# Cappucciyes/ViT-With-OpenCL

Hardware: AMD Instinct MI355X
Metric: images/sec ViT-B/16 224x224 bs512 (higher is better)
Workload: dtype f32

## Files before the change

vit-with-opencl_amd/csrc/ViT_hip.c:

```c
#include "ViT_opencl.h"
#include "vit_ingest.h"
#include "vit_plan.h"

#include <math.h>
#include <pthread.h>
#include <stddef.h>
#include <stdint.h>
#include <stdio.h>
#include <stdlib.h>
#include <string.h>
#include <time.h>

#define TRY(expr)                 \
    do {                          \
        int try_rc_ = (expr);     \
        if (try_rc_ != 0) {       \
            rc = try_rc_;         \
            goto fail;            \
        }                         \
    } while (0)

enum { DESC_RING = 8 };

enum { FEAT_NONE, FEAT_DEVICE, FEAT_HOST };

struct staged
{
    void *dev, *pinned[2];
    char *host;
    size_t per_image;
};

struct vit_hip_ctx
{
    vit_config cfg;
    int device;
    int max_batch;
    int n_tensors;
    vh_stream_t stream;

    struct vit_plan plan;

    void *slab[N_SLABS];
    float **w;
    struct operand *op;

    float *x;
    float *y;
    float *attn;
    float *qkv;
    float *hid;
    float *stats;
    float *cls;
    float *d_logits;
    float *d_probs;
    float *d_images[2];
    float *h_images[2];
    float *h_logits[2];
    float *h_probs[2];
    vh_stream_t copy_stream;
    vh_event_t up_done[2], comp_done[2], out_done[2];

    vh_resize_desc *h_desc[DESC_RING];
    vh_resize_desc *d_desc[DESC_RING];
    vh_event_t desc_done[DESC_RING];
    int desc_live[DESC_RING];
    int desc_next;

    struct feature_req
    {
        int form;
        vit_feature_spec spec;
        int layer[4];
        vit_feature_buffers out;
        struct staged st[2];
    } feat;

    struct topk_req
    {
        int form;
        vit_topk_spec spec;
        vit_topk_buffers out;
        struct staged st[2];
    } topk;

    struct attn_req
    {
        int form;
        vit_attn_spec spec;
        int layer[4];
        vit_attn_buffers out;
        struct staged st[2];
    } amap;
    const struct attn_req *attn_serving;

    vh_event_t *prof_ev;
    int *prof_class;
    int prof_cap;
    int prof_used;
    unsigned prof_mask;
};

static int prof_begin(vit_hip_ctx *ctx, vh_stream_t s, int op_class)
{
    if (!ctx->prof_ev || ctx->prof_used >= ctx->prof_cap)
        return -1;
    if (ctx->prof_mask && !(ctx->prof_mask & (1u << op_class)))
        return -1;
    const int slot = ctx->prof_used++;
    ctx->prof_class[slot] = op_class;
    vh_event_record(ctx->prof_ev[2 * slot], s);
    return slot;
}

// ... 34 lines not shown
const vit_config *vit_hip_config(const vit_hip_ctx *ctx) { return &ctx->cfg; }
int vit_hip_device(const vit_hip_ctx *ctx) { return ctx->device; }
float *vit_hip_logits_buffer(vit_hip_ctx *ctx) { return ctx->d_logits; }
vh_stream_t vit_hip_stream(const vit_hip_ctx *ctx) { return ctx->stream; }
int vit_hip_max_batch(const vit_hip_ctx *ctx) { return ctx->max_batch; }
const float *vit_hip_weight(const vit_hip_ctx *ctx, int idx)
{
    return (idx >= 0 && idx < ctx->n_tensors) ? ctx->w[idx] : NULL;
}

static int staged_alloc(const vit_hip_ctx *ctx, struct staged *st)
{
    const size_t bytes = (size_t)ctx->max_batch * st->per_image;
    int rc = vh_malloc(&st->dev, bytes);
    for (int slot = 0; slot < 2 && rc == 0; ++slot)
        rc = vh_host_alloc(&st->pinned[slot], bytes);
    return rc;
}

static void staged_release(struct staged *st)
{
    if (st->dev) vh_free(st->dev);
    st->dev = NULL;
    for (int slot = 0; slot < 2; ++slot) {
        if (st->pinned[slot]) vh_host_free(st->pinned[slot]);
        st->pinned[slot] = NULL;
    }
}

static int staged_d2h(const vit_hip_ctx *ctx, const struct staged *st, int slot, int m)
{
    return vh_d2h(st->pinned[slot], st->dev, (size_t)m * st->per_image, ctx->stream);
}

static void staged_scatter(const struct staged *st, int slot, int first, int m)
{
    memcpy(st->host + (size_t)first * st->per_image, st->pinned[slot], (size_t)m * st->per_image);
}

static void request_release(struct staged st[2])
{
    staged_release(&st[0]);
    staged_release(&st[1]);
}

void vit_hip_destroy(vit_hip_ctx *ctx)
{
    if (!ctx)
        return;
    if (ctx->stream) {
        vh_set_device(ctx->device);
        vh_stream_sync(ctx->stream);
    }
    prof_release(ctx);
    request_release(ctx->feat.st);
    request_release(ctx->topk.st);
    request_release(ctx->amap.st);
    for (int i = 0; i < N_SLABS; ++i)
        if (ctx->slab[i])
            vh_free(ctx->slab[i]);
    float *dev[] = {ctx->x, ctx->y, ctx->attn, ctx->qkv, ctx->hid, ctx->stats,
                    ctx->cls, ctx->d_logits, ctx->d_probs, ctx->d_images[0], ctx->d_images[1]};
    for (size_t i = 0; i < sizeof(dev) / sizeof(dev[0]); ++i)
        if (dev[i])
            vh_free(dev[i]);
    float *host[] = {ctx->h_images[0], ctx->h_images[1], ctx->h_logits[0], ctx->h_logits[1],
                     ctx->h_probs[0], ctx->h_probs[1]};
    for (size_t i = 0; i < sizeof(host) / sizeof(host[0]); ++i)
        if (host[i])
            vh_host_free(host[i]);
    for (int i = 0; i < DESC_RING; ++i) {
        if (ctx->d_desc[i]) vh_free(ctx->d_desc[i]);
        if (ctx->h_desc[i]) vh_host_free(ctx->h_desc[i]);
        if (ctx->desc_done[i]) vh_event_destroy(ctx->desc_done[i]);
    }
    for (int i = 0; i < 2; ++i) {
        if (ctx->up_done[i]) vh_event_destroy(ctx->up_done[i]);
        if (ctx->comp_done[i]) vh_event_destroy(ctx->comp_done[i]);
        if (ctx->out_done[i]) vh_event_destroy(ctx->out_done[i]);
    }
    if (ctx->copy_stream)
        vh_stream_destroy(ctx->copy_stream);
    if (ctx->stream)
        vh_stream_destroy(ctx->stream);
    free(ctx->w);
    free(ctx->op);
    free(ctx);
}

static float **layer_tensors(const vit_hip_ctx *ctx, int l) { return ctx->w + 4 + 12 * l; }

static int alloc_weights(vit_hip_ctx *ctx)
{
    int rc = 0;
    for (int i = 0; i < N_SLABS; ++i)
        if (ctx->plan.slab_bytes[i])
            TRY(vh_malloc(&ctx->slab[i], ctx->plan.slab_bytes[i]));
    plan_layout(&ctx->plan, &ctx->cfg, ctx->slab, ctx->w, ctx->op, NULL);
    return 0;
fail:
    return rc;
}

static int fill_weights(vit_hip_ctx *ctx, const Network *networks)
{
    int rc = 0;
// ... 1049 lines not shown
        return 1;
    TRY(vh_set_device(ctx->device));
    TRY(vh_stream_sync(ctx->stream));
    prof_release(ctx);
    if (max_forwards <= 0)
        return 0;
    const int per_forward = 1 + 7 * ctx->cfg.depth + 3 + 4 + 1 + 4;
    ctx->prof_cap = per_forward * max_forwards;
    ctx->prof_ev = (vh_event_t *)calloc((size_t)2 * ctx->prof_cap, sizeof(vh_event_t));
    ctx->prof_class = (int *)calloc((size_t)ctx->prof_cap, sizeof(int));
    if (!ctx->prof_ev || !ctx->prof_class) {
        prof_release(ctx);
        return 4;
    }
    for (int i = 0; i < 2 * ctx->prof_cap; ++i)
        TRY(vh_event_create(&ctx->prof_ev[i]));
    return 0;
fail:
    prof_release(ctx);
    return rc;
}

int vit_hip_profile_select(vit_hip_ctx *ctx, unsigned op_mask)
{
    if (!ctx)
        return 1;
    ctx->prof_mask = op_mask;
    return 0;
}

int vit_hip_profile_read(vit_hip_ctx *ctx, double ms_sum[VIT_OP_COUNT], long launches[VIT_OP_COUNT])
{
    int rc = 0;
    if (!ctx || !ms_sum || !launches)
        return 1;
    TRY(vh_set_device(ctx->device));
    for (int k = 0; k < VIT_OP_COUNT; ++k) {
        ms_sum[k] = 0.0;
        launches[k] = 0;
    }
    for (int i = 0; i < ctx->prof_used; ++i) {
        float ms = 0.0f;
        TRY(vh_event_sync(ctx->prof_ev[2 * i + 1]));
        TRY(vh_event_elapsed_ms(&ms, ctx->prof_ev[2 * i], ctx->prof_ev[2 * i + 1]));
        ms_sum[ctx->prof_class[i]] += ms;
        launches[ctx->prof_class[i]] += 1;
    }
    ctx->prof_used = 0;
    return 0;
fail:
    return rc;
}

static void scatter_outputs(vit_hip_ctx *ctx, int slot, int first, int m, const struct staged *const *arrays, int n_arrays, float **probs)
{
    const size_t NC = (size_t)ctx->cfg.num_classes;
    for (int a = 0; a < n_arrays; ++a)
        staged_scatter(arrays[a], slot, first, m);
    if (probs)
        for (int i = 0; i < m; ++i)
            memcpy(probs[first + i], ctx->h_probs[slot] + (size_t)i * NC, NC * sizeof(float));
}

struct gather_job
{
    char *dst;
    const struct ingest_src *src;
    const struct ingest_plan *plan;
    int first, count;
    int base;
    size_t per_image;
};

static void *gather_worker(void *arg)
{
    const struct gather_job *j = (const struct gather_job *)arg;
    for (int i = j->first; i < j->first + j->count; ++i) {
        if (j->plan) {
            ingest_pack(j->dst, j->plan, j->src, i);
            continue;
        }
        const void *from = j->src->kind == INGEST_F32 ? (const void *)j->src->host_f32[j->base + i].data
                                                      : (const void *)(j->src->u8 + (size_t)(j->base + i) * j->per_image);
        memcpy(j->dst + (size_t)i * j->per_image, from, j->per_image);
    }
    return NULL;
}

static void gather_images(void *dst, const struct ingest_src *src, const struct ingest_plan *plan, int base, int m, size_t per_image)
{
    enum { MAX_THREADS = 8 };
    int nt = m / 16;
    if (nt > MAX_THREADS)
        nt = MAX_THREADS;
    struct gather_job jobs[MAX_THREADS];
    pthread_t tid[MAX_THREADS];
    int started = 0;
    if (nt < 2) {
        struct gather_job all = {.dst = (char *)dst, .src = src, .plan = plan, .first = 0, .count = m, .base = base, .per_image = per_image};
        gather_worker(&all);
        return;
    }
    const int per = (m + nt - 1) / nt;
    for (int t = 0; t < nt; ++t) {
        const int first = t * per, count = first >= m ? 0 : (m - first < per ? m - first : per);
        jobs[t] = (struct gather_job){.dst = (char *)dst, .src = src, .plan = plan, .first = first, .count = count, .base = base, .per_image = per_image};
        if (count == 0)
            break;
        if (t == nt - 1 || pthread_create(&tid[started], NULL, gather_worker, &jobs[t]) != 0)
            gather_worker(&jobs[t]);
        else
            ++started;
    }
    for (int t = 0; t < started; ++t)
        pthread_join(tid[t], NULL);
}

static int forward_pipelined(vit_hip_ctx *ctx, const struct ingest_src *src, struct ingest_plan *plan, int n, float *logits, float **probs,
                             int form)
{
    int rc = 0;
    const struct feature_req *fr;
    const struct topk_req *tk;
    const struct attn_req *ar;
    if (armed_requests(ctx, "forward", form, &fr, &tk, &ar))
        return 1;
    TRY(vh_set_device(ctx->device));
    const vit_config *c = &ctx->cfg;
    const size_t bytes = (size_t)c->in_chans * c->img_size * c->img_size * (src->kind == INGEST_F32 ? sizeof(float) : 1);
    const size_t NC = (size_t)c->num_classes;
    const struct staged logits_st = {ctx->d_logits, {ctx->h_logits[0], ctx->h_logits[1]}, (char *)logits, NC * sizeof(float)};
    const struct staged *arrays[7];
    int n_arrays = 0;
    if (logits)
        arrays[n_arrays++] = &logits_st;
    for (int a = 0; a < 6; ++a) {
        const struct staged *st = a < 2 ? (fr ? &fr->st[a] : NULL) : a < 4 ? (tk ? &tk->st[a - 2] : NULL) : (ar ? &ar->st[a - 4] : NULL);
        if (st && st->dev)
            arrays[n_arrays++] = st;
    }

    int prev_first = 0, prev_m = 0, k = 0;
    for (int first = 0, m = 0; first < n; first += m, ++k) {
        const int s = k & 1;
        struct ingest_src dev = *src;
        dev.on_device = 1;
        m = (n - first < ctx->max_batch) ? n - first : ctx->max_batch;
        size_t up = (size_t)m * bytes;
        int jobs = m;
        switch (src->kind) {
        case INGEST_F32:
            dev.host_f32 = NULL;
            dev.f32 = ctx->d_images[s];
            break;
        case INGEST_U8:
            dev.u8 = (const unsigned char *)ctx->d_images[s];
            break;
        default:
            m = ingest_plan_chunk(plan, src, first, n, (const unsigned char *)ctx->d_images[s]);
            up = plan->bytes;
            jobs = plan->n_src;
            dev.items = plan->items;
        }
        if (m <= 0) {
            rc = vh_set_error(1, "forward: an image does not fit a staging slot");
            goto fail;
        }
        gather_images(ctx->h_images[s], src, plan, first, jobs, bytes);
        if (k >= 2)
            TRY(vh_stream_wait_event(ctx->copy_stream, ctx->comp_done[s]));
        TRY(vh_h2d(ctx->d_images[s], ctx->h_images[s], up, ctx->copy_stream));
        TRY(vh_event_record(ctx->up_done[s], ctx->copy_stream));

        TRY(vh_stream_wait_event(ctx->stream, ctx->up_done[s]));
        TRY(forward_device(ctx, &dev, m, ctx->d_logits, probs ? ctx->d_probs : NULL, ctx->stream, fr, tk, ar));
        TRY(vh_event_record(ctx->comp_done[s], ctx->stream));
        int a = 0;
        if (logits)
            TRY(staged_d2h(ctx, arrays[a++], s, m));
        if (probs)
            TRY(vh_d2h(ctx->h_probs[s], ctx->d_probs, (size_t)m * NC * sizeof(float), ctx->stream));
        for (; a < n_arrays; ++a)
            TRY(staged_d2h(ctx, arrays[a], s, m));
        TRY(vh_event_record(ctx->out_done[s], ctx->stream));

        if (k >= 1) {
            TRY(vh_event_sync(ctx->out_done[s ^ 1]));
            scatter_outputs(ctx, s ^ 1, prev_first, prev_m, arrays, n_arrays, probs);
        }
        prev_first = first;
        prev_m = m;
    }
    TRY(vh_event_sync(ctx->out_done[(k - 1) & 1]));
    scatter_outputs(ctx, (k - 1) & 1, prev_first, prev_m, arrays, n_arrays, probs);
    return 0;
fail:
    vh_stream_sync(ctx->copy_stream);
    vh_stream_sync(ctx->stream);
    return rc;
}

static int forward_host_images(vit_hip_ctx *ctx, const ImageData *images, int n, float *logits, float **probs, int form)
{
    if (!ctx || !images || n <= 0)
        return 1;
    const vit_config *c = &ctx->cfg;
    for (int i = 0; i < n; ++i)
        if (!images[i].data || images[i].c != c->in_chans || images[i].h != c->img_size ||
            images[i].w != c->img_size)
            return 5;
    const struct ingest_src src = {.kind = INGEST_F32, .host_f32 = images};
    return forward_pipelined(ctx, &src, NULL, n, logits, probs, form);
}

int vit_hip_forward(vit_hip_ctx *ctx, const ImageData *images, int n, float *logits, float **probs)
{
    return forward_host_images(ctx, images, n, logits, probs, FEAT_HOST);
}

static int forward_host_u8(vit_hip_ctx *ctx, const char *who, const struct ingest_src *src, int n, float *logits, float **probs)
{
    if (source_check(who, ctx, src, n))
        return 1;
    struct ingest_plan *plan = NULL;
    if (src->kind != INGEST_U8) {
        const struct ingest_model model = model_of(ctx);
        if (!(plan = ingest_plan_new(&model, src->kind)))
            return ingest_refuse(who, "out of host memory");
    }
    const int rc = forward_pipelined(ctx, src, plan, n, logits, probs, FEAT_HOST);
    ingest_plan_free(plan);
    return rc;
}

int vit_hip_forward_u8(vit_hip_ctx *ctx, const unsigned char *images, int n, int layout,
                       const vit_pixel_norm *norm, float *logits, float **probs)
{
    const struct ingest_src src = {.kind = INGEST_U8, .u8 = images, .layout = layout, .norm = norm};
    return forward_host_u8(ctx, "vit_hip_forward_u8", &src, n, logits, probs);
}

int vit_hip_forward_u8_resized(vit_hip_ctx *ctx, const vit_image_u8 *images, int n, int layout, const vit_resize_crop *rc,
                               const vit_pixel_norm *norm, float *logits, float **probs)
{
    const struct ingest_src src = {.kind = INGEST_U8_RESIZED, .images = images, .rc = rc, .layout = layout, .norm = norm};
    return forward_host_u8(ctx, "vit_hip_forward_u8_resized", &src, n, logits, probs);
}
// ... 287 lines not shown
```

vit-with-opencl_amd/csrc/vit_plan.c:

```c
#include "vit_plan.h"
#include "vit_ingest.h"

#include <stdio.h>
#include <stdlib.h>
#include <string.h>

void plan_env_parse(struct plan_env *env, const char *const v[PLAN_ENV_COUNT])
{
    const char *const p = v[PLAN_ENV_PRECISION], *const fold = v[PLAN_ENV_LN_FOLD], *const attn = v[PLAN_ENV_ATTN];
    env->precision = (p && p[0] == 'b') ? VIT_PRECISION_BF16_GEMM
                   : (p && strncmp(p, "fp16x2", 6) == 0) ? VIT_PRECISION_F32_FP16X2
                   : (p && strncmp(p, "fp8", 3) == 0) ? VIT_PRECISION_FP8_GEMM : VIT_PRECISION_F32;
    env->p3_off = v[PLAN_ENV_P3] && v[PLAN_ENV_P3][0] == '0';
    env->fp32_native = v[PLAN_ENV_GEMM_FP32] && v[PLAN_ENV_GEMM_FP32][0] == 'n';
    env->ln_fold = (fold && fold[0] == '0') ? 0 : (fold && fold[0] == '1') ? 1 : -1;
    env->last_layer_cls = v[PLAN_ENV_LAST_LAYER] && strcmp(v[PLAN_ENV_LAST_LAYER], "cls") == 0;
    env->attn_long = attn && strcmp(attn, "long") == 0;
    env->attn_tiled = attn && attn[0] == 't';
}

void plan_env_read(struct plan_env *env)
{
    const char *const values[PLAN_ENV_COUNT] = {getenv("VIT_HIP_PRECISION"), getenv("VIT_HIP_P3"), getenv("VIT_HIP_GEMM_FP32"),
                                                getenv("VIT_HIP_LN_FOLD"), getenv("VIT_HIP_LAST_LAYER"), getenv("VIT_HIP_ATTN")};
    plan_env_parse(env, values);
}

static size_t max_of(size_t a, size_t b) { return a > b ? a : b; }

size_t plan_cls_only_scratch(const vit_config *cfg, int n, size_t off[3])
{
    const size_t rows = (size_t)n, E = (size_t)cfg->embed_dim, F = (size_t)cfg->mlp_hidden;
    size_t o[3];
    o[0] = align_up(rows * E * 4, 256);
    o[1] = o[0] + align_up(rows * E * 6, 256);
    o[2] = o[1] + align_up(rows * E * 6, 256);
    if (off)
        memcpy(off, o, sizeof o);
    return o[2] + rows * F * 6;
}

static void *place(void *slab, size_t *off, size_t bytes)
{
    void *p = slab ? (char *)slab + *off : NULL;
    *off += align_up(bytes, 256);
    return p;
}

void plan_layout(const struct vit_plan *plan, const vit_config *cfg, void *const slabs[N_SLABS], float **w, struct operand *op,
                 size_t bytes[N_SLABS])
{
    void *const none[N_SLABS] = {NULL};
    void *const *slab = slabs ? slabs : none;
    struct operand unplaced_op;
    size_t off[N_SLABS] = {0};
    for (int i = 0; i < vit_config_num_tensors(cfg); ++i) {
        float *p = (float *)place(slab[SLAB_F32], &off[SLAB_F32], vit_config_tensor_size(cfg, i) * sizeof(float));
        if (slabs)
            w[i] = p;
    }
    for (int m = 0; m < 4 * cfg->depth; ++m) {
        struct operand *o = slabs ? &op[m] : &unplaced_op;
        const size_t cnt = vit_config_tensor_size(cfg, plan_operand_tensor(m));
        o->w = place(slab[SLAB_OPERAND], &off[SLAB_OPERAND], cnt * (size_t)plan->operand_bytes);
        if (plan->operand_scales)
            o->scales = place(slab[SLAB_OPERAND], &off[SLAB_OPERAND], cnt / 32);
        if (plan->ln_fold && m % 2 == 0) {
            const size_t nb = vit_config_tensor_size(cfg, plan_operand_tensor(m) + 1) * sizeof(float);
            o->colsum = (float *)place(slab[SLAB_FOLD], &off[SLAB_FOLD], nb);
            o->bias_folded = (float *)place(slab[SLAB_FOLD], &off[SLAB_FOLD], nb);
        }
    }
    place(slab[SLAB_CONV], &off[SLAB_CONV],
          (size_t)vh_patch_planes_k(cfg->in_chans, cfg->patch_size) * (size_t)cfg->embed_dim * 2 * (size_t)plan->conv_parts);
    if (bytes)
        memcpy(bytes, off, sizeof(off));
}

static void plan_arena(struct vit_plan *plan, const vit_config *cfg, int max_batch)
{
    const size_t E = (size_t)cfg->embed_dim, F = (size_t)cfg->mlp_hidden, act = (size_t)plan->act_bytes, n = (size_t)max_batch;
    const size_t rows = n * (size_t)plan->tokens, grid = (size_t)(cfg->img_size / cfg->patch_size);
    const size_t img = (size_t)cfg->in_chans * cfg->img_size * cfg->img_size;
    const int fp8 = plan->precision == VIT_PRECISION_FP8_GEMM, resizes = cfg->in_chans <= 4;
    const int planes_path = plan->use_p3 || plan->precision == VIT_PRECISION_BF16_GEMM || fp8;
    size_t b;

    plan->x_bytes = rows * E * sizeof(float);

    b = rows * E * act;
    if (fp8) {
        plan->e_scales_off = align_up(rows * E, 256);
// ... 108 lines not shown
```

vit-with-opencl_amd/csrc/vit_plan.h:

```cpp
#ifndef VIT_PLAN_H
#define VIT_PLAN_H

#include "ViT_opencl.h"

#include <stddef.h>

struct operand
{
    void *w;
    void *scales;
    float pair_scale;
    float *colsum, *bias_folded;
};

enum { SLAB_F32, SLAB_OPERAND, SLAB_CONV, SLAB_FOLD, N_SLABS };

enum { ATTN_STREAMING, ATTN_HD64, ATTN_HD80, ATTN_LONG };

enum { STREAMING_MAX_TOKENS = 512 };

enum { MAX_DEPTH = 256, MAX_TENSORS = 4 + 12 * MAX_DEPTH + 4 };

static inline int plan_operand_tensor(int m)
{
    static const int big[4] = {2, 4, 8, 10};
    return 4 + 12 * (m / 4) + big[m % 4];
}

struct plan_env
{
    int precision;
    int p3_off;
    int fp32_native;
    int ln_fold;
    int last_layer_cls;
    int attn_long;
    int attn_tiled;
};
enum { PLAN_ENV_PRECISION, PLAN_ENV_P3, PLAN_ENV_GEMM_FP32, PLAN_ENV_LN_FOLD, PLAN_ENV_LAST_LAYER, PLAN_ENV_ATTN, PLAN_ENV_COUNT };
void plan_env_parse(struct plan_env *env, const char *const values[PLAN_ENV_COUNT]);
void plan_env_read(struct plan_env *env);

struct vit_plan
{
    int precision;
    int ln_fold;
    int use_p3;
    int cls_only_last;
    int attn_form;
    int fp32_native;
    int attn_rows_streaming;
    int tokens;
    int qkv_form;
    int weight_planes;
    int operand_bytes;
    int operand_scales;
    int conv_parts;
    int planes_patch_embed;
    int act_bytes;
    int cls_only_ok;
    size_t slab_bytes[N_SLABS];
    size_t x_bytes, y_bytes, attn_bytes, qkv_bytes, ws_bytes, stats_bytes;
    size_t crop_off;
    size_t e_scales_off, hid_scales_off;
};

int plan_make(struct vit_plan *plan, const vit_config *cfg, int n_tensors, int max_batch, int precision, int ln_fold,
              const struct plan_env *env);

void plan_layout(const struct vit_plan *plan, const vit_config *cfg, void *const slabs[N_SLABS], float **w, struct operand *op,
                 size_t bytes[N_SLABS]);

size_t plan_cls_only_scratch(const vit_config *cfg, int n, size_t off[3]);

#endif
```

vit-with-opencl_amd/csrc/attention_p3.hip:

```cpp
#include "kernelHandler.h"
#include "vit_kernels.h"
#include "fp32_split.h"
#include "gemm_common.h"

namespace {

constexpr int HD = 64;
constexpr int MAX_LDS = 160 * 1024;
constexpr int MAX_ROWS = 208;

typedef const __attribute__((address_space(1))) void *gptr_t;
typedef __attribute__((address_space(3))) void *lptr_t;
typedef short s16x4 __attribute__((ext_vector_type(4)));

template <int NKT, int NPL, int OUTK>
__global__ __launch_bounds__(64 * NKT) void attention_p3_kernel(const char *__restrict__ qkv3, char *__restrict__ out3,
                                                               unsigned char *__restrict__ out_scales,
                                                               int T, int E, int H, int n_items, int RB)
{
    static_assert((NPL == 3 && OUTK == 3) || (NPL == 1 && (OUTK == 4 || OUTK == 0 || OUTK == 8)), "parts / output kind");
    typedef typename PartT<NPL>::type part_t;
    constexpr int NT = NPL == 3 ? 6 : 1;
    extern __shared__ __attribute__((aligned(16))) char smem[];
    const int slot = 2 * NPL * RB * 64;
    char *Kb = smem, *Vb = smem + slot;

    const int tid = threadIdx.x, lane = tid & 63;
    const int wave = __builtin_amdgcn_readfirstlane(tid >> 6);
    const int lr = lane & 31, lh = lane >> 5;
    const int E32 = E >> 5, rb16 = RB >> 4, pieces = 2 * NPL * rb16;
    const size_t prow = (size_t)(n_items / H) * T;

    auto dma = [&](int item, int which , char *dst) {
        const int b = item / H, h = item - b * H;
        const int ks0 = which * E32 + 2 * h;
        for (int p = wave; p < pieces; p += NKT) {
            const int gp = p / rb16, rb = p - gp * rb16;
            const int r = 16 * rb + (lane >> 2);
            int c = lane & 3;
            if (which == 1)
                c ^= swz64(lane >> 4);
            const char *src = qkv3 + ((size_t)(ks0 * NPL + gp) * prow + (size_t)b * T + min(r, T - 1)) * 64 + 16 * c;
            __builtin_amdgcn_global_load_lds((gptr_t)src, (lptr_t)(dst + p * 1024), 16, 0, 0);
        }
    };

    const int q = wave * 32 + lr;
    part_t qp[HD / 16][NPL];
    auto load_q = [&](int item) {
        const int b = item / H, h = item - b * H;
        const size_t row = (size_t)b * T + min(q, T - 1);
#pragma unroll
        for (int g = 0; g < HD / 16; ++g)
#pragma unroll
            for (int pl = 0; pl < NPL; ++pl)
                qp[g][pl] = __builtin_bit_cast(part_t, *reinterpret_cast<const f32x4 *>(
                                qkv3 + ((size_t)((2 * h + (g >> 1)) * NPL + pl) * prow + row) * 64 + 16 * (2 * (g & 1) + lh)));
    };

    int kofs[2], kofs_last[2];
    {
        const int rl = min(32 * (NKT - 1) + lr, RB - 1);
#pragma unroll
        for (int gl = 0; gl < 2; ++gl) {
            kofs[gl] = lr * 64 + 16 * ((2 * gl + lh) ^ swz64(lr >> 2));
            kofs_last[gl] = rl * 64 + 16 * ((2 * gl + lh) ^ swz64(rl >> 2));
        }
    }
    const int vofs = (4 * lh + ((lane & 15) >> 2)) * 64 + ((lane & 16) + 4 * (lane & 3)) * 2;

    int item = blockIdx.x;
    if (item >= n_items)
        return;
    load_q(item);
    dma(item, 1, Kb);
    __syncthreads();

    for (; item < n_items; item += gridDim.x) {
        const int b = item / H, h = item - b * H;
        const int next = item + gridDim.x;
        dma(item, 2, Vb);

        f32x16 s[NKT];
        part_t kp[3][NPL];
        auto read_k = [&](part_t (&k3)[NPL], int f) {
            const int j = f / (HD / 16), g = f % (HD / 16);
#pragma unroll
            for (int o = 0; o < NPL; ++o) {
                const int pl = (NPL - o) % NPL;
                const char *base = Kb + ((g >> 1) * NPL + pl) * RB * 64;
                k3[pl] = __builtin_bit_cast(part_t, (j < NKT - 1)
                    ? *reinterpret_cast<const f32x4 *>(base + kofs[g & 1] + j * 32 * 64)
                    : *reinterpret_cast<const f32x4 *>(base + kofs_last[g & 1]));
            }
        };
        read_k(kp[0], 0);
        if (NKT * (HD / 16) > 1)
            read_k(kp[1], 1);
#pragma unroll
        for (int f = 0; f < NKT * (HD / 16); ++f) {
            const int j = f / (HD / 16), g = f % (HD / 16);
            if (g == 0) {
#pragma unroll
                for (int r = 0; r < 16; ++r)
                    s[j][r] = 0.0f;
            }
            if (f + 2 < NKT * (HD / 16))
                read_k(kp[(f + 2) % 3], f + 2);
#pragma unroll
            for (int t = 0; t < NT; ++t)
                s[j] = mfma_part(kp[f % 3][term_w<NPL>(t)], qp[g][term_a<NPL>(t)], s[j]);
            if (NPL == 3) {
#pragma unroll
                for (int r = 0; r < 3; ++r) {
                    __builtin_amdgcn_sched_group_barrier(0x100, 1, 0);
                    __builtin_amdgcn_sched_group_barrier(0x008, 2, 0);
                }
                __builtin_amdgcn_sched_barrier(0);
            }
        }

        __syncthreads();
        if (next < n_items) {
            dma(next, 1, Kb);
            load_q(next);
        }

#pragma unroll
        for (int r = 0; r < 16; ++r) {
            const int key = 32 * (NKT - 1) + (r & 3) + 8 * (r >> 2) + 4 * lh;
            s[NKT - 1][r] = key < T ? s[NKT - 1][r] : -INFINITY;
        }
        float mx = -INFINITY;
#pragma unroll
        for (int j = 0; j < NKT; ++j)
#pragma unroll
            for (int r = 0; r < 16; ++r)
                mx = fmaxf(mx, s[j][r]);
        mx = fmaxf(mx, __shfl_xor(mx, 32));
        const float c1 = 1.44269504088896340736f / sqrtf((float)HD);
        const float c2 = -mx * c1;
        float sum = 0.0f;
#pragma unroll
        for (int j = 0; j < NKT; ++j)
#pragma unroll
            for (int r = 0; r < 16; ++r) {
                const float e = __builtin_amdgcn_exp2f(__builtin_fmaf(s[j][r], c1, c2));
                s[j][r] = e;
                sum += e;
            }
        sum += __shfl_xor(sum, 32);
        const float inv_sum = 1.0f / sum;
#pragma unroll
        for (int j = 0; j < NKT; ++j)
#pragma unroll
            for (int r = 0; r < 16; ++r)
                s[j][r] = s[j][r] * inv_sum;

        f32x16 o[2];
#pragma unroll
        for (int r = 0; r < 16; ++r) {
            o[0][r] = 0.0f;
            o[1][r] = 0.0f;
        }
        part_t vq[2][NPL], pp[NPL];
        auto read_v = [&](part_t (&v3)[NPL], int f) {
            const int j = f >> 2, t = (f >> 1) & 1, dt = f & 1;
            const int r0 = (j == NKT - 1) ? min(32 * j + 16 * t, RB - 16) : 32 * j + 16 * t;
#pragma unroll
            for (int o3 = 0; o3 < NPL; ++o3) {
                const int pl = (NPL - o3) % NPL;
                const char *vp = Vb + (dt * NPL + pl) * RB * 64 + r0 * 64 + vofs;
                const s16x4 lo = __builtin_amdgcn_ds_read_tr16_b64_v4i16((__attribute__((address_space(3))) s16x4 *)(vp));
                const s16x4 hi = __builtin_amdgcn_ds_read_tr16_b64_v4i16((__attribute__((address_space(3))) s16x4 *)(vp + 8 * 64));
                typedef short s16x8 __attribute__((ext_vector_type(8)));
                v3[pl] = __builtin_bit_cast(part_t, s16x8{lo[0], lo[1], lo[2], lo[3], hi[0], hi[1], hi[2], hi[3]});
            }
        };
        read_v(vq[0], 0);
#pragma unroll
        for (int f = 0; f < 4 * NKT; ++f) {
            const int j = f >> 2, t = (f >> 1) & 1, dt = f & 1;
            if (f + 1 < 4 * NKT)
                read_v(vq[(f + 1) & 1], f + 1);
            if (dt == 0)
                split_parts(f32x4{s[j][8 * t], s[j][8 * t + 1], s[j][8 * t + 2], s[j][8 * t + 3]},
                            f32x4{s[j][8 * t + 4], s[j][8 * t + 5], s[j][8 * t + 6], s[j][8 * t + 7]}, pp);
            if (!(j == NKT - 1 && 32 * j + 16 * t >= T)) {
#pragma unroll
                for (int tt = 0; tt < NT; ++tt)
                    o[dt] = mfma_part(vq[f & 1][term_w<NPL>(tt)], pp[term_a<NPL>(tt)], o[dt]);
            }
        }

        if (q < T) {
            typedef unsigned u32x2 __attribute__((ext_vector_type(2)));
            typedef unsigned u32x4 __attribute__((ext_vector_type(4)));
            constexpr int OPL = OUTK == 3 ? 3 : 1;
#pragma unroll
            for (int dt = 0; dt < 2; ++dt) {
                if (OUTK == 0) {
                    float *row = reinterpret_cast<float *>(out3) + ((size_t)b * T + q) * E + h * HD + 32 * dt + 4 * lh;
#pragma unroll
                    for (int g = 0; g < 4; ++g)
                        *reinterpret_cast<f32x4 *>(row + 8 * g) = f32x4{o[dt][4 * g], o[dt][4 * g + 1], o[dt][4 * g + 2], o[dt][4 * g + 3]};
                    continue;
                }
                if (OUTK == 8) {
                    float amax = 0.0f;
#pragma unroll
                    for (int r = 0; r < 16; ++r)
                        amax = fmaxf(amax, fabsf(o[dt][r]));
                    amax = fmaxf(amax, __shfl_xor(amax, 32));
                    unsigned sbyte;
                    float mult;
                    mx_block_scale(amax, sbyte, mult);
                    unsigned x[4];
#pragma unroll
                    for (int g = 0; g < 4; ++g)
                        x[g] = pack_fp8x4(f32x4{o[dt][4 * g], o[dt][4 * g + 1], o[dt][4 * g + 2], o[dt][4 * g + 3]} * mult);
                    const auto r02 = __builtin_amdgcn_permlane32_swap(x[0], x[2], false, false);
                    const auto r13 = __builtin_amdgcn_permlane32_swap(x[1], x[3], false, false);
                    const int col = h * HD + 32 * dt, ks = col >> 7, blk = (col >> 5) & 3;
                    const size_t row = (size_t)b * T + q;
                    *reinterpret_cast<u32x4 *>(out3 + ((size_t)ks * prow + row) * 128 + 32 * blk + 16 * lh) =
                        u32x4{r02[0], r02[1], r13[0], r13[1]};
                    if (lh == 0)
                        out_scales[mx_act_scale_index(ks, blk, row, prow)] = (unsigned char)sbyte;
                    continue;
                }
                u32x2 pg[4][OPL];
#pragma unroll
                for (int g = 0; g < 4; ++g) {
                    bf16x4 part[3];
                    const f32x4 v4 = f32x4{o[dt][4 * g], o[dt][4 * g + 1], o[dt][4 * g + 2], o[dt][4 * g + 3]};
                    if (OUTK == 3) {
                        split4(v4, part[0], part[1], part[2]);
                    } else {
#pragma unroll
                        for (int e = 0; e < 4; ++e)
                            part[0][e] = (__bf16)v4[e];
                    }
#pragma unroll
                    for (int pl = 0; pl < OPL; ++pl)
                        pg[g][pl] = __builtin_bit_cast(u32x2, part[pl]);
                }
                char *d3 = out3 + ((size_t)(2 * h + dt) * OPL * prow + (size_t)b * T + q) * 64 + 16 * lh;
#pragma unroll
                for (int pl = 0; pl < OPL; ++pl)
#pragma unroll
                    for (int g = 0; g < 4; g += 2) {
                        const auto r0 = __builtin_amdgcn_permlane32_swap(pg[g][pl][0], pg[g + 1][pl][0], false, false);
                        const auto r1 = __builtin_amdgcn_permlane32_swap(pg[g][pl][1], pg[g + 1][pl][1], false, false);
                        *reinterpret_cast<u32x4 *>(d3 + (size_t)pl * prow * 64 + 16 * g) = u32x4{r0[0], r1[0], r0[1], r1[1]};
                    }
            }
        }

        __syncthreads();
    }
}

template <int NKT, int NPL, int OUTK>
int launch_k(hipStream_t st, const char *qkv3, char *out3, unsigned char *out_scales, int n_images, int T, int E, int H)
{
    const int RB = (T + 15) / 16 * 16;
    const size_t lds = (size_t)2 * 2 * NPL * RB * 64;
    VH_SET_LDS_ONCE((attention_p3_kernel<NKT, NPL, OUTK>), MAX_LDS);
    const int num_cus = vh_device_cus(vh_current_device());
    const int n_items = n_images * H;
    const int grid = n_items < num_cus ? n_items : num_cus;
    hipLaunchKernelGGL((attention_p3_kernel<NKT, NPL, OUTK>), dim3(grid), dim3(64 * NKT), lds, st, qkv3, out3, out_scales, T, E, H, n_items, RB);
    VH_LAUNCH_CHECK("attention_p3_kernel");
    return 0;
}


template <int NPL, int OUTK>
int launch_t(hipStream_t st, const char *in, char *out, unsigned char *out_scales, int n_images, int tokens, int embed_dim, int num_heads)
{
    switch ((tokens + 31) / 32) {
    case 1: return launch_k<1, NPL, OUTK>(st, in, out, out_scales, n_images, tokens, embed_dim, num_heads);
    case 2: return launch_k<2, NPL, OUTK>(st, in, out, out_scales, n_images, tokens, embed_dim, num_heads);
    case 3: return launch_k<3, NPL, OUTK>(st, in, out, out_scales, n_images, tokens, embed_dim, num_heads);
    case 4: return launch_k<4, NPL, OUTK>(st, in, out, out_scales, n_images, tokens, embed_dim, num_heads);
    case 5: return launch_k<5, NPL, OUTK>(st, in, out, out_scales, n_images, tokens, embed_dim, num_heads);
    case 6: return launch_k<6, NPL, OUTK>(st, in, out, out_scales, n_images, tokens, embed_dim, num_heads);
    default: return launch_k<7, NPL, OUTK>(st, in, out, out_scales, n_images, tokens, embed_dim, num_heads);
    }
}

int check_args(const char *who, const void *in, const void *out, int n_images, int tokens, int embed_dim, int num_heads)
{
    if (!in || !out)
        return vh_fail(1, "%s: null pointer argument", who);
    if (n_images <= 0 || tokens <= 0 || num_heads <= 0 || embed_dim != num_heads * HD || tokens > MAX_ROWS)
        return vh_fail(1, "%s: needs head_dim 64 and 1 <= tokens <= %d (n=%d tokens=%d embed=%d heads=%d)", who,
                       MAX_ROWS, n_images, tokens, embed_dim, num_heads);
    if ((((uintptr_t)in | (uintptr_t)out) & 15) != 0)
        return vh_fail(1, "%s: pointers must be 16-byte aligned", who);
    return 0;
}

}

extern "C" int vh_launch_attention_planes(vh_stream_t s, const void *qkv_planes, void *out_planes, int n_images,
                                          int tokens, int embed_dim, int num_heads)
{
    if (int rc = check_args("vh_launch_attention_planes", qkv_planes, out_planes, n_images, tokens, embed_dim, num_heads))
        return rc;
    return launch_t<3, 3>((hipStream_t)s, static_cast<const char *>(qkv_planes), static_cast<char *>(out_planes), nullptr,
                          n_images, tokens, embed_dim, num_heads);
}

extern "C" int vh_launch_attention_planes_f16(vh_stream_t s, const void *qkv_planes_f16, void *output, int output_planes,
                                              int n_images, int tokens, int embed_dim, int num_heads)
{
    if (int rc = check_args("vh_launch_attention_planes_f16", qkv_planes_f16, output, n_images, tokens, embed_dim, num_heads))
        return rc;
    const char *in = static_cast<const char *>(qkv_planes_f16);
// ... 16 lines not shown
```

Before: 6087.

## Use persistent host gather pool and ramp chunk sizes to start GPU sooner

Per-chunk pthread creation for image gathering is replaced by a persistent worker pool that pulls work items through an atomic counter. Chunk sizes now ramp geometrically from a small first chunk (sized from a 40 MiB byte budget) up to max_batch, so the first upload and compute can begin before a full batch is gathered. The wait on the previous compute is also moved ahead of the gather. The cost being targeted is thread-spawn overhead and the unhidden host gather plus H2D at pipeline start. In exchange, more and smaller chunks mean more kernel launches and smaller GEMMs during the ramp.

```diff
diff --git a/vit-with-opencl_amd/csrc/ViT_hip.c b/vit-with-opencl_amd/csrc/ViT_hip.c
--- a/vit-with-opencl_amd/csrc/ViT_hip.c
+++ b/vit-with-opencl_amd/csrc/ViT_hip.c
@@ -1,6 +1,7 @@
 #include "ViT_opencl.h"
 #include "vit_ingest.h"
 #include "vit_plan.h"
+#include "vit_pool.h"
 
 #include <math.h>
 #include <pthread.h>
@@ -60,6 +61,7 @@
     float *h_probs[2];
     vh_stream_t copy_stream;
     vh_event_t up_done[2], comp_done[2], out_done[2];
+    struct vit_pool pool;
 
     vh_resize_desc *h_desc[DESC_RING];
     vh_resize_desc *d_desc[DESC_RING];
@@ -200,6 +202,7 @@
         vh_set_device(ctx->device);
         vh_stream_sync(ctx->stream);
     }
+    vit_pool_stop(&ctx->pool);
     prof_release(ctx);
     request_release(ctx->feat.st);
     request_release(ctx->topk.st);
@@ -1355,6 +1358,8 @@
     return rc;
 }
 
+enum { HOST_WORKERS = 7 };
+
 static void scatter_outputs(vit_hip_ctx *ctx, int slot, int first, int m, const struct staged *const *arrays, int n_arrays, float **probs)
 {
     const size_t NC = (size_t)ctx->cfg.num_classes;
@@ -1370,53 +1375,62 @@
     char *dst;
     const struct ingest_src *src;
     const struct ingest_plan *plan;
-    int first, count;
     int base;
     size_t per_image;
 };
 
-static void *gather_worker(void *arg)
+static void gather_item(void *arg, int item)
 {
     const struct gather_job *j = (const struct gather_job *)arg;
-    for (int i = j->first; i < j->first + j->count; ++i) {
-        if (j->plan) {
-            ingest_pack(j->dst, j->plan, j->src, i);
-            continue;
-        }
-        const void *from = j->src->kind == INGEST_F32 ? (const void *)j->src->host_f32[j->base + i].data
-                                                      : (const void *)(j->src->u8 + (size_t)(j->base + i) * j->per_image);
-        memcpy(j->dst + (size_t)i * j->per_image, from, j->per_image);
-    }
-    return NULL;
-}
-
-static void gather_images(void *dst, const struct ingest_src *src, const struct ingest_plan *plan, int base, int m, size_t per_image)
-{
-    enum { MAX_THREADS = 8 };
-    int nt = m / 16;
-    if (nt > MAX_THREADS)
-        nt = MAX_THREADS;
-    struct gather_job jobs[MAX_THREADS];
-    pthread_t tid[MAX_THREADS];
-    int started = 0;
-    if (nt < 2) {
-        struct gather_job all = {.dst = (char *)dst, .src = src, .plan = plan, .first = 0, .count = m, .base = base, .per_image = per_image};
-        gather_worker(&all);
+    const int i = item;
+    if (j->plan) {
+        ingest_pack(j->dst, j->plan, j->src, i);
         return;
     }
-    const int per = (m + nt - 1) / nt;
-    for (int t = 0; t < nt; ++t) {
-        const int first = t * per, count = first >= m ? 0 : (m - first < per ? m - first : per);
-        jobs[t] = (struct gather_job){.dst = (char *)dst, .src = src, .plan = plan, .first = first, .count = count, .base = base, .per_image = per_image};
-        if (count == 0)
-            break;
-        if (t == nt - 1 || pthread_create(&tid[started], NULL, gather_worker, &jobs[t]) != 0)
-            gather_worker(&jobs[t]);
-        else
-            ++started;
-    }
-    for (int t = 0; t < started; ++t)
-        pthread_join(tid[t], NULL);
+    const void *from = j->src->kind == INGEST_F32 ? (const void *)j->src->host_f32[j->base + i].data
+                                                  : (const void *)(j->src->u8 + (size_t)(j->base + i) * j->per_image);
+    memcpy(j->dst + (size_t)i * j->per_image, from, j->per_image);
+}
+
+struct chunk
+{
+    int first, m, slot;
+    struct ingest_src dev;
+};
+
+static int stage_chunk(vit_hip_ctx *ctx, const struct ingest_src *src, struct ingest_plan *plan, int k, int first, int n, int ramp_first,
+                       size_t bytes, struct chunk *ch)
+{
+    int rc = 0;
+    const int s = k & 1;
+    ch->first = first;
+    ch->slot = s;
+    ch->dev = *src;
+    ch->dev.on_device = 1;
+    ch->m = plan_chunk_size(k, n - first, ctx->max_batch, ramp_first);
+    switch (src->kind) {
+    case INGEST_F32:
+        ch->dev.host_f32 = NULL;
+        ch->dev.f32 = ctx->d_images[s];
+        break;
+    case INGEST_U8:
+        ch->dev.u8 = (const unsigned char *)ctx->d_images[s];
+        break;
+    default:
+        ch->m = ingest_plan_chunk(plan, src, first, n, (const unsigned char *)ctx->d_images[s]);
+        ch->dev.items = plan->items;
+    }
+    if (ch->m <= 0)
+        return vh_set_error(1, "forward: an image does not fit a staging slot");
+    if (k >= 2)
+        TRY(vh_stream_wait_event(ctx->copy_stream, ctx->comp_done[s]));
+    const struct gather_job job = {.dst = (char *)ctx->h_images[s], .src = src, .plan = plan, .base = first, .per_image = bytes};
+    vit_pool_run(&ctx->pool, gather_item, (void *)&job, plan ? plan->n_src : ch->m, plan ? 2 : 4);
+    TRY(vh_h2d(ctx->d_images[s], ctx->h_images[s], plan ? plan->bytes : (size_t)ch->m * bytes, ctx->copy_stream));
+    TRY(vh_event_record(ctx->up_done[s], ctx->copy_stream));
+    return 0;
+fail:
+    return rc;
 }
 
 static int forward_pipelined(vit_hip_ctx *ctx, const struct ingest_src *src, struct ingest_plan *plan, int n, float *logits, float **probs,
@@ -1432,6 +1446,7 @@
     const vit_config *c = &ctx->cfg;
     const size_t bytes = (size_t)c->in_chans * c->img_size * c->img_size * (src->kind == INGEST_F32 ? sizeof(float) : 1);
     const size_t NC = (size_t)c->num_classes;
+    const int ramp_first = plan ? ctx->max_batch : plan_chunk_first(ctx->max_batch, bytes);
     const struct staged logits_st = {ctx->d_logits, {ctx->h_logits[0], ctx->h_logits[1]}, (char *)logits, NC * sizeof(float)};
     const struct staged *arrays[7];
     int n_arrays = 0;
@@ -1442,41 +1457,14 @@
         if (st && st->dev)
             arrays[n_arrays++] = st;
     }
-
-    int prev_first = 0, prev_m = 0, k = 0;
-    for (int first = 0, m = 0; first < n; first += m, ++k) {
-        const int s = k & 1;
-        struct ingest_src dev = *src;
-        dev.on_device = 1;
-        m = (n - first < ctx->max_batch) ? n - first : ctx->max_batch;
-        size_t up = (size_t)m * bytes;
-        int jobs = m;
-        switch (src->kind) {
-        case INGEST_F32:
-            dev.host_f32 = NULL;
-            dev.f32 = ctx->d_images[s];
-            break;
-        case INGEST_U8:
-            dev.u8 = (const unsigned char *)ctx->d_images[s];
-            break;
-        default:
-            m = ingest_plan_chunk(plan, src, first, n, (const unsigned char *)ctx->d_images[s]);
-            up = plan->bytes;
-            jobs = plan->n_src;
-            dev.items = plan->items;
-        }
-        if (m <= 0) {
-            rc = vh_set_error(1, "forward: an image does not fit a staging slot");
-            goto fail;
-        }
-        gather_images(ctx->h_images[s], src, plan, first, jobs, bytes);
-        if (k >= 2)
-            TRY(vh_stream_wait_event(ctx->copy_stream, ctx->comp_done[s]));
-        TRY(vh_h2d(ctx->d_images[s], ctx->h_images[s], up, ctx->copy_stream));
-        TRY(vh_event_record(ctx->up_done[s], ctx->copy_stream));
-
+    vit_pool_start(&ctx->pool, HOST_WORKERS);
+
+    struct chunk cur = {0}, prev = {0};
+    for (int k = 0, first = 0; first < n; first += cur.m, ++k) {
+        TRY(stage_chunk(ctx, src, plan, k, first, n, ramp_first, bytes, &cur));
+        const int s = cur.slot, m = cur.m;
         TRY(vh_stream_wait_event(ctx->stream, ctx->up_done[s]));
-        TRY(forward_device(ctx, &dev, m, ctx->d_logits, probs ? ctx->d_probs : NULL, ctx->stream, fr, tk, ar));
+        TRY(forward_device(ctx, &cur.dev, m, ctx->d_logits, probs ? ctx->d_probs : NULL, ctx->stream, fr, tk, ar));
         TRY(vh_event_record(ctx->comp_done[s], ctx->stream));
         int a = 0;
         if (logits)
@@ -1488,14 +1476,13 @@
         TRY(vh_event_record(ctx->out_done[s], ctx->stream));
 
         if (k >= 1) {
-            TRY(vh_event_sync(ctx->out_done[s ^ 1]));
-            scatter_outputs(ctx, s ^ 1, prev_first, prev_m, arrays, n_arrays, probs);
+            TRY(vh_event_sync(ctx->out_done[prev.slot]));
+            scatter_outputs(ctx, prev.slot, prev.first, prev.m, arrays, n_arrays, probs);
         }
-        prev_first = first;
-        prev_m = m;
-    }
-    TRY(vh_event_sync(ctx->out_done[(k - 1) & 1]));
-    scatter_outputs(ctx, (k - 1) & 1, prev_first, prev_m, arrays, n_arrays, probs);
+        prev = cur;
+    }
+    TRY(vh_event_sync(ctx->out_done[prev.slot]));
+    scatter_outputs(ctx, prev.slot, prev.first, prev.m, arrays, n_arrays, probs);
     return 0;
 fail:
     vh_stream_sync(ctx->copy_stream);
diff --git a/vit-with-opencl_amd/csrc/vit_plan.c b/vit-with-opencl_amd/csrc/vit_plan.c
--- a/vit-with-opencl_amd/csrc/vit_plan.c
+++ b/vit-with-opencl_amd/csrc/vit_plan.c
@@ -38,6 +38,24 @@
     if (off)
         memcpy(off, o, sizeof o);
     return o[2] + rows * F * 6;
+}
+
+int plan_chunk_first(int max_batch, size_t bytes_per_image)
+{
+    if (max_batch <= 0 || bytes_per_image == 0)
+        return max_batch > 0 ? max_batch : 1;
+    size_t first = (size_t)CHUNK_RAMP_BYTES / bytes_per_image / 32 * 32;
+    if (first < 32)
+        first = 32;
+    return first * CHUNK_RAMP_MIN_STEPS <= (size_t)max_batch ? (int)first : max_batch;
+}
+
+int plan_chunk_size(int k, int left, int max_batch, int first)
+{
+    int m = max_batch > 0 ? max_batch : 1;
+    if (first >= 1 && first < m && k >= 0 && k < 31 && ((long long)first << k) < (long long)m)
+        m = (int)((long long)first << k);
+    return left < m ? (left > 0 ? left : 1) : m;
 }
 
 static void *place(void *slab, size_t *off, size_t bytes)
diff --git a/vit-with-opencl_amd/csrc/vit_plan.h b/vit-with-opencl_amd/csrc/vit_plan.h
--- a/vit-with-opencl_amd/csrc/vit_plan.h
+++ b/vit-with-opencl_amd/csrc/vit_plan.h
@@ -73,4 +73,10 @@
 
 size_t plan_cls_only_scratch(const vit_config *cfg, int n, size_t off[3]);
 
+enum { CHUNK_RAMP_BYTES = 40 << 20, CHUNK_RAMP_MIN_STEPS = 4 };
+
+int plan_chunk_first(int max_batch, size_t bytes_per_image);
+
+int plan_chunk_size(int k, int left, int max_batch, int first);
+
 #endif
diff --git a/vit-with-opencl_amd/csrc/vit_pool.c b/vit-with-opencl_amd/csrc/vit_pool.c
--- /dev/null
+++ b/vit-with-opencl_amd/csrc/vit_pool.c
@@ -0,0 +1,105 @@
+#include "vit_pool.h"
+
+static void take_items(struct vit_pool *p, vit_pool_fn fn, void *arg, int count)
+{
+    for (int i; (i = atomic_fetch_add(&p->next, 1)) < count;)
+        fn(arg, i);
+}
+
+static void *pool_worker(void *arg)
+{
+    struct vit_pool *p = (struct vit_pool *)arg;
+    unsigned long seen = 0;
+    pthread_mutex_lock(&p->mu);
+    for (;;) {
+        while (!p->stop && p->job == seen)
+            pthread_cond_wait(&p->wake, &p->mu);
+        if (p->stop)
+            break;
+        seen = p->job;
+        const vit_pool_fn fn = p->fn;
+        void *const fn_arg = p->arg;
+        const int count = p->count;
+        pthread_mutex_unlock(&p->mu);
+        take_items(p, fn, fn_arg, count);
+        pthread_mutex_lock(&p->mu);
+        if (--p->busy == 0)
+            pthread_cond_signal(&p->idle);
+    }
+    pthread_mutex_unlock(&p->mu);
+    return NULL;
+}
+
+int vit_pool_start(struct vit_pool *p, int n_workers)
+{
+    if (p->n_workers > 0)
+        return p->n_workers;
+    if (n_workers > VIT_POOL_MAX_WORKERS)
+        n_workers = VIT_POOL_MAX_WORKERS;
+    if (n_workers <= 0)
+        return 0;
+    if (pthread_mutex_init(&p->mu, NULL) != 0)
+        return 0;
+    if (pthread_cond_init(&p->wake, NULL) != 0) {
+        pthread_mutex_destroy(&p->mu);
+        return 0;
+    }
+    if (pthread_cond_init(&p->idle, NULL) != 0) {
+        pthread_cond_destroy(&p->wake);
+        pthread_mutex_destroy(&p->mu);
+        return 0;
+    }
+    p->stop = 0;
+    p->job = 0;
+    p->busy = 0;
+    atomic_init(&p->next, 0);
+    int started = 0;
+    while (started < n_workers && pthread_create(&p->tid[started], NULL, pool_worker, p) == 0)
+        ++started;
+    p->n_workers = started;
+    if (started == 0) {
+        pthread_cond_destroy(&p->idle);
+        pthread_cond_destroy(&p->wake);
+        pthread_mutex_destroy(&p->mu);
+    }
+    return started;
+}
+
+void vit_pool_run(struct vit_pool *p, vit_pool_fn fn, void *arg, int count, int min_parallel)
+{
+    if (p->n_workers == 0 || count < min_parallel || count < 2) {
+        for (int i = 0; i < count; ++i)
+            fn(arg, i);
+        return;
+    }
+    pthread_mutex_lock(&p->mu);
+    p->fn = fn;
+    p->arg = arg;
+    p->count = count;
+    atomic_store(&p->next, 0);
+    p->busy = p->n_workers;
+    ++p->job;
+    pthread_cond_broadcast(&p->wake);
+    pthread_mutex_unlock(&p->mu);
+    take_items(p, fn, arg, count);
+    pthread_mutex_lock(&p->mu);
+    while (p->busy > 0)
+        pthread_cond_wait(&p->idle, &p->mu);
+    pthread_mutex_unlock(&p->mu);
+}
+
+void vit_pool_stop(struct vit_pool *p)
+{
+    if (p->n_workers == 0)
+        return;
+    pthread_mutex_lock(&p->mu);
+    p->stop = 1;
+    pthread_cond_broadcast(&p->wake);
+    pthread_mutex_unlock(&p->mu);
+    for (int t = 0; t < p->n_workers; ++t)
+        pthread_join(p->tid[t], NULL);
+    p->n_workers = 0;
+    pthread_cond_destroy(&p->idle);
+    pthread_cond_destroy(&p->wake);
+    pthread_mutex_destroy(&p->mu);
+}
diff --git a/vit-with-opencl_amd/csrc/vit_pool.h b/vit-with-opencl_amd/csrc/vit_pool.h
--- /dev/null
+++ b/vit-with-opencl_amd/csrc/vit_pool.h
@@ -0,0 +1,32 @@
+#ifndef VIT_POOL_H
+#define VIT_POOL_H
+
+#include <pthread.h>
+#include <stdatomic.h>
+
+enum { VIT_POOL_MAX_WORKERS = 7 };
+
+typedef void (*vit_pool_fn)(void *arg, int item);
+
+struct vit_pool
+{
+    pthread_mutex_t mu;
+    pthread_cond_t wake, idle;
+    pthread_t tid[VIT_POOL_MAX_WORKERS];
+    int n_workers;
+    int stop;
+    unsigned long job;
+    int busy;
+    vit_pool_fn fn;
+    void *arg;
+    int count;
+    atomic_int next;
+};
+
+int vit_pool_start(struct vit_pool *p, int n_workers);
+
+void vit_pool_run(struct vit_pool *p, vit_pool_fn fn, void *arg, int count, int min_parallel);
+
+void vit_pool_stop(struct vit_pool *p);
+
+#endif
```

New measurement: 6092 (median of 4 runs). No clear change (+0.1%).

## Pipeline softmax normalization into P split and restructure attention PV loop

Applied to the files above, without the earlier changes.

Folds the 1/sum normalization into a new split_p4 helper that scales and splits probabilities into bf16/fp16 parts just before each MFMA, and software-pipelines the split one step ahead of the products. Makes the LDS slot size a compile-time constant (RS) and limits the K/V DMA to at most four waves. The tail block is peeled and skipped when it lies beyond T. These aim to drop a separate normalization pass, overlap VALU splitting with MFMA, and cut DMA issue overhead, but they add code complexity and shift the rounding of the split parts.

```diff
diff --git a/vit-with-opencl_amd/csrc/attention_p3.hip b/vit-with-opencl_amd/csrc/attention_p3.hip
--- a/vit-with-opencl_amd/csrc/attention_p3.hip
+++ b/vit-with-opencl_amd/csrc/attention_p3.hip
@@ -13,6 +13,39 @@
 typedef __attribute__((address_space(3))) void *lptr_t;
 typedef short s16x4 __attribute__((ext_vector_type(4)));
 
+__device__ __forceinline__ void split_p4(const f32x4 &u, float k, bf16x8 (&o)[3], int e0)
+{
+    typedef float f32x2 __attribute__((ext_vector_type(2)));
+    typedef __bf16 bf16x2 __attribute__((ext_vector_type(2)));
+#pragma unroll
+    for (int e = 0; e < 4; e += 2) {
+        float x0 = u[e] * k, x1 = u[e + 1] * k;
+        asm("" : "+v"(x0));
+        asm("" : "+v"(x1));
+        const bf16x2 h = __builtin_convertvector(f32x2{x0, x1}, bf16x2);
+        float a0 = x0 - (float)h[0], a1 = x1 - (float)h[1];
+        asm("" : "+v"(a0));
+        asm("" : "+v"(a1));
+        const bf16x2 m = __builtin_convertvector(f32x2{a0, a1}, bf16x2);
+        float b0 = a0 - (float)m[0], b1 = a1 - (float)m[1];
+        asm("" : "+v"(b0));
+        asm("" : "+v"(b1));
+        const bf16x2 l = __builtin_convertvector(f32x2{b0, b1}, bf16x2);
+        o[0][e0 + e] = h[0], o[0][e0 + e + 1] = h[1];
+        o[1][e0 + e] = m[0], o[1][e0 + e + 1] = m[1];
+        o[2][e0 + e] = l[0], o[2][e0 + e + 1] = l[1];
+    }
+}
+__device__ __forceinline__ void split_p4(const f32x4 &u, float k, half8 (&o)[1], int e0)
+{
+#pragma unroll
+    for (int e = 0; e < 4; ++e) {
+        float x = u[e] * k;
+        asm("" : "+v"(x));
+        o[0][e0 + e] = (_Float16)x;
+    }
+}
+
 template <int NKT, int NPL, int OUTK>
 __global__ __launch_bounds__(64 * NKT) void attention_p3_kernel(const char *__restrict__ qkv3, char *__restrict__ out3,
                                                                unsigned char *__restrict__ out_scales,
@@ -22,7 +55,8 @@
     typedef typename PartT<NPL>::type part_t;
     constexpr int NT = NPL == 3 ? 6 : 1;
     extern __shared__ __attribute__((aligned(16))) char smem[];
-    const int slot = 2 * NPL * RB * 64;
+    constexpr int RS = 32 * NKT < MAX_ROWS ? 32 * NKT : MAX_ROWS;
+    constexpr int slot = 2 * NPL * RS * 64;
     char *Kb = smem, *Vb = smem + slot;
 
     const int tid = threadIdx.x, lane = tid & 63;
@@ -34,14 +68,17 @@
     auto dma = [&](int item, int which , char *dst) {
         const int b = item / H, h = item - b * H;
         const int ks0 = which * E32 + 2 * h;
-        for (int p = wave; p < pieces; p += NKT) {
+        constexpr int NL = NKT >= 5 ? 4 : NKT;
+        if (wave >= NL)
+            return;
+        for (int p = wave; p < pieces; p += NL) {
             const int gp = p / rb16, rb = p - gp * rb16;
             const int r = 16 * rb + (lane >> 2);
             int c = lane & 3;
             if (which == 1)
                 c ^= swz64(lane >> 4);
             const char *src = qkv3 + ((size_t)(ks0 * NPL + gp) * prow + (size_t)b * T + min(r, T - 1)) * 64 + 16 * c;
-            __builtin_amdgcn_global_load_lds((gptr_t)src, (lptr_t)(dst + p * 1024), 16, 0, 0);
+            __builtin_amdgcn_global_load_lds((gptr_t)src, (lptr_t)(dst + (gp * (RS / 16) + rb) * 1024), 16, 0, 0);
         }
     };
 
@@ -60,7 +97,7 @@
 
     int kofs[2], kofs_last[2];
     {
-        const int rl = min(32 * (NKT - 1) + lr, RB - 1);
+        const int rl = min(32 * (NKT - 1) + lr, RS - 1);
 #pragma unroll
         for (int gl = 0; gl < 2; ++gl) {
             kofs[gl] = lr * 64 + 16 * ((2 * gl + lh) ^ swz64(lr >> 2));
@@ -88,7 +125,7 @@
 #pragma unroll
             for (int o = 0; o < NPL; ++o) {
                 const int pl = (NPL - o) % NPL;
-                const char *base = Kb + ((g >> 1) * NPL + pl) * RB * 64;
+                const char *base = Kb + ((g >> 1) * NPL + pl) * RS * 64;
                 k3[pl] = __builtin_bit_cast(part_t, (j < NKT - 1)
                     ? *reinterpret_cast<const f32x4 *>(base + kofs[g & 1] + j * 32 * 64)
                     : *reinterpret_cast<const f32x4 *>(base + kofs_last[g & 1]));
@@ -151,11 +188,6 @@
             }
         sum += __shfl_xor(sum, 32);
         const float inv_sum = 1.0f / sum;
-#pragma unroll
-        for (int j = 0; j < NKT; ++j)
-#pragma unroll
-            for (int r = 0; r < 16; ++r)
-                s[j][r] = s[j][r] * inv_sum;
 
         f32x16 o[2];
 #pragma unroll
@@ -163,34 +195,48 @@
             o[0][r] = 0.0f;
             o[1][r] = 0.0f;
         }
-        part_t vq[2][NPL], pp[NPL];
+        part_t vq[2][NPL], pq[2][NPL];
         auto read_v = [&](part_t (&v3)[NPL], int f) {
             const int j = f >> 2, t = (f >> 1) & 1, dt = f & 1;
-            const int r0 = (j == NKT - 1) ? min(32 * j + 16 * t, RB - 16) : 32 * j + 16 * t;
+            const int r0 = min(32 * j + 16 * t, RS - 16);
 #pragma unroll
             for (int o3 = 0; o3 < NPL; ++o3) {
                 const int pl = (NPL - o3) % NPL;
-                const char *vp = Vb + (dt * NPL + pl) * RB * 64 + r0 * 64 + vofs;
+                const char *vp = Vb + (dt * NPL + pl) * RS * 64 + r0 * 64 + vofs;
                 const s16x4 lo = __builtin_amdgcn_ds_read_tr16_b64_v4i16((__attribute__((address_space(3))) s16x4 *)(vp));
                 const s16x4 hi = __builtin_amdgcn_ds_read_tr16_b64_v4i16((__attribute__((address_space(3))) s16x4 *)(vp + 8 * 64));
                 typedef short s16x8 __attribute__((ext_vector_type(8)));
                 v3[pl] = __builtin_bit_cast(part_t, s16x8{lo[0], lo[1], lo[2], lo[3], hi[0], hi[1], hi[2], hi[3]});
             }
         };
+        auto split_quarter = [&](int hh, int qd) {
+            const int j = hh >> 1, r = 8 * (hh & 1) + 4 * qd;
+            split_p4(f32x4{s[j][r], s[j][r + 1], s[j][r + 2], s[j][r + 3]}, inv_sum, pq[hh & 1], 4 * qd);
+        };
+        auto products = [&](int f) {
+#pragma unroll
+            for (int tt = 0; tt < NT; ++tt)
+                o[f & 1] = mfma_part(vq[f & 1][term_w<NPL>(tt)], pq[(f >> 1) & 1][term_a<NPL>(tt)], o[f & 1]);
+        };
+        constexpr int LAST = 2 * NKT - 1;
         read_v(vq[0], 0);
-#pragma unroll
-        for (int f = 0; f < 4 * NKT; ++f) {
-            const int j = f >> 2, t = (f >> 1) & 1, dt = f & 1;
-            if (f + 1 < 4 * NKT)
+        split_quarter(0, 0);
+        split_quarter(0, 1);
+#pragma unroll
+        for (int f = 0; f < 2 * LAST; ++f) {
+            if (f + 1 < 2 * LAST)
                 read_v(vq[(f + 1) & 1], f + 1);
-            if (dt == 0)
-                split_parts(f32x4{s[j][8 * t], s[j][8 * t + 1], s[j][8 * t + 2], s[j][8 * t + 3]},
-                            f32x4{s[j][8 * t + 4], s[j][8 * t + 5], s[j][8 * t + 6], s[j][8 * t + 7]}, pp);
-            if (!(j == NKT - 1 && 32 * j + 16 * t >= T)) {
-#pragma unroll
-                for (int tt = 0; tt < NT; ++tt)
-                    o[dt] = mfma_part(vq[f & 1][term_w<NPL>(tt)], pp[term_a<NPL>(tt)], o[dt]);
-            }
+            if ((f >> 1) + 1 < LAST)
+                split_quarter((f >> 1) + 1, f & 1);
+            products(f);
+        }
+        if (32 * (NKT - 1) + 16 < T) {
+            read_v(vq[0], 2 * LAST);
+            read_v(vq[1], 2 * LAST + 1);
+            split_quarter(LAST, 0);
+            split_quarter(LAST, 1);
+            products(2 * LAST);
+            products(2 * LAST + 1);
         }
 
         if (q < T) {
@@ -265,7 +311,7 @@
 int launch_k(hipStream_t st, const char *qkv3, char *out3, unsigned char *out_scales, int n_images, int T, int E, int H)
 {
     const int RB = (T + 15) / 16 * 16;
-    const size_t lds = (size_t)2 * 2 * NPL * RB * 64;
+    const size_t lds = (size_t)2 * 2 * NPL * (32 * NKT < MAX_ROWS ? 32 * NKT : MAX_ROWS) * 64;
     VH_SET_LDS_ONCE((attention_p3_kernel<NKT, NPL, OUTK>), MAX_LDS);
     const int num_cus = vh_device_cus(vh_current_device());
     const int n_items = n_images * H;
```

After: 6075 before, 6083 after (median of 6 runs). Within noise of the previous version (+0.1%).
